# medical-genomics-group/ci-gwas

Hardware: AMD Instinct MI355X
Metric: ci_tests_per_sec (higher is better)
Workload: dtype f32; 1 GPU; cusk level sweep, one LD block 10000 SNPs x 20 traits, N=16384, alpha=0.0001, max level 5 (north_star headline); correlation matrix from synthetic .bed (Kendall-npn/Pearson) resident in HBM; n_variables=10020, engine=cusk

## Files before the change

ci-gwas_amd/csrc/cusk_internal.h:

```cpp
#pragma once
#include <hip/hip_runtime.h>

#include <cstdint>
#include <cstdio>
#include <string>
#include <vector>

#include "../../include/cusk_hip.h"

namespace cusk {

constexpr int kML = CUSK_ML;
constexpr int kLevels = CUSK_ML + 2;
constexpr unsigned long long kNone = ~0ull;
constexpr int kNumClasses = 5;
constexpr int kClassCap[kNumClasses] = {39, 63, 127, 191, 1 << 30};
constexpr int kThreads = 256;
constexpr int kTmajMinLevelDefault = 6;
constexpr int kCounterSlots = 512;
constexpr size_t kLdsLimit = 160 * 1024;

struct DevBuf
{
    void *p = nullptr;
// ... 75 lines not shown

    int n = 0;
    int words = 0;
    int mode = -1;
    bool have_result = false;
    cusk::DevBuf adj, adj0;
    cusk::DevBuf deg, binom, counters, slots, rec_base, ti, queue, symflag;
    cusk::DevBuf off[2], nbr[2], best[2];
    cusk::DevBuf planblk;
    unsigned plan_seq = 0;
    cusk::DevBuf off1;
    cusk::DevBuf items[2][cusk::kNumClasses];
    cusk::DevBuf rec_x, rec_y, rec_l, rec_s;
    long long rec_cap = 0;
    long long rec_slots = 0;
    cusk::DevBuf den_x, den_y, den_l, den_z, den_s, den_counts, den_off;
    long long den_stride = 0;
    bool records_ready = false, z_ready = false;
    cusk::DevBuf scratch_a, scratch_b;
    const float *last_C = nullptr;
    int last_levels = 0;
    std::vector<int> batch_lo, batch_hi;
    cusk::DevBuf row_range, row_blk, blk_woff;
    cusk::PinnedBuf batch_pinned;
    cusk::PinnedBuf res_pinned;
    cusk::DevBuf rv, rpos, sel, wpre;
    cusk::DevBuf nv;
    int level1_form = -1;
    long long nrec = 0;
    cusk::LevelCounters *hcnt = nullptr;
    unsigned long long *hslots = nullptr;
    long long *hrec_base = nullptr;
    unsigned long long *hcanon = nullptr;
    int *hflag = nullptr;
    std::vector<unsigned long long> binom_host;
    long long binom_rows = 0;
    cusk::HostGate *hgate = nullptr, *hgate_dev = nullptr;
    int run_seq = 0;
    long long item_cap_cur = 0;
    hipEvent_t ev_main[2] = {nullptr, nullptr};
    hipEvent_t ev_run[2] = {nullptr, nullptr};
    hipEvent_t ev_k0[cusk::kLevels], ev_k1[cusk::kLevels], ev_l0[cusk::kLevels], ev_l1[cusk::kLevels];

    int opt_fast = 1;
    int opt_validate = 0;
    int opt_het_filter = 0;
    int opt_het_rows = 0;
    int opt_corr_fp4 = 1;
    int opt_pair = 1;
    int opt_rows = 1;
    int opt_vec = 1;
    int opt_overlap = 1;
    int opt_corr_popcount = 0;
    int opt_corr_mxp_f32 = 0;
    int opt_assume_symmetric = 0;
    long long opt_queue_cap = 4ll << 20;
    int opt_hostprof = 0;
    int opt_tmaj_validate_stride = 1;
    int opt_max_staged_classes = -1;
    int opt_tmaj_min_level = cusk::kTmajMinLevelDefault;
    long long opt_chunk = 2048;
    long long opt_chunk0 = 512;
    long long opt_chunk0_low = 256;
    int opt_vec_threads = 64;
    long long opt_item_cap = 1ll << 20;
    int opt_lookahead = 2;
    int opt_sync2 = 1;
    int opt_l1_threads = 0;
    int opt_l1_lds_row = 1;
    int opt_timing = 1;
    long long opt_sep_ws_budget = 4ll << 30;

    int shard_rank = 0, shard_world = 1;
    int shard_host_staging = 0;
    cusk_exchange_fn shard_fn = nullptr;
    void *shard_user = nullptr;
    cusk::PinnedBuf shard_host;

    cusk::DevBuf bed_dev, phen_dev, mean_dev, std_dev, planes, mxp_dev, pxp_dev, mxp_bq;
    cusk::DevBuf pc_masks, pc_counts;
    cusk::DevBuf mp_bits;
    cusk::DevBuf corr_tab[2];
    cusk::PinnedBuf corr_tab_pinned[2];
    hipEvent_t ev_corr[5] = {nullptr, nullptr, nullptr, nullptr, nullptr};
    float corr_ms[4] = {0, 0, 0, 0};
    float prune_ms[5] = {0, 0, 0, 0, 0};
    float ord_ms[3] = {0, 0, 0};
    hipEvent_t ev_prune[6] = {nullptr, nullptr, nullptr, nullptr, nullptr, nullptr};
    float phen_ms[5] = {0, 0, 0, 0, 0};
};

namespace cusk {

inline int fail(cusk_engine *e, int code, const std::string &msg)
{
    if (e) e->err = msg;
    return code;
}

#define CUSK_HIP(e, call)                                                                        \
// ... 48 lines not shown
```

ci-gwas_amd/csrc/engine.hip:

```cpp
#include <algorithm>
#include <cstdlib>
#include <cstring>

#include "sweep_common.h"

using namespace cusk;


extern "C" int cusk_engine_create(cusk_engine **out, int device, void *stream)
{
    if (!out) return CUSK_ERR_ARG;
    *out = nullptr;
    int ndev = 0;
    if (hipGetDeviceCount(&ndev) != hipSuccess || ndev <= 0)
    {
        std::fprintf(stderr, "libcusk_hip: no HIP device available (this library has no CPU fallback)\n");
        return CUSK_ERR_HIP;
    }
    if (device < 0 || device >= ndev) return CUSK_ERR_ARG;
    if (hipSetDevice(device) != hipSuccess) return CUSK_ERR_HIP;
    cusk_engine *e = new cusk_engine();
    e->device = device;
    for (int l = 0; l < kLevels; l++) e->ev_k0[l] = e->ev_k1[l] = e->ev_l0[l] = e->ev_l1[l] = nullptr;
    bool ok = true;
    if (stream)
    {
        e->stream = reinterpret_cast<hipStream_t>(stream);
        e->own_stream = false;
    }
    else
    {
        ok = ok && hipStreamCreateWithFlags(&e->stream, hipStreamNonBlocking) == hipSuccess;
        e->own_stream = ok;
    }
    ok = ok && hipStreamCreateWithFlags(&e->stream2, hipStreamNonBlocking) == hipSuccess;
    ok = ok && hipStreamCreateWithFlags(&e->stream3, hipStreamNonBlocking) == hipSuccess;
    ok = ok && hipEventCreateWithFlags(&e->ev_fork, hipEventDisableTiming) == hipSuccess;
    ok = ok && hipEventCreateWithFlags(&e->ev_join, hipEventDisableTiming) == hipSuccess;
    ok = ok && hipEventCreateWithFlags(&e->ev_z, hipEventDisableTiming) == hipSuccess;
    {
        char *hctl = nullptr;
        ok = ok && hipHostMalloc(reinterpret_cast<void **>(&hctl), kCtlBytes) == hipSuccess;
        if (ok)
        {
            e->hcnt = reinterpret_cast<LevelCounters *>(hctl + kCtlCnt);
            e->hslots = reinterpret_cast<unsigned long long *>(hctl + kCtlSlots);
            e->hrec_base = reinterpret_cast<long long *>(hctl + kCtlRecBase);
            e->hcanon = reinterpret_cast<unsigned long long *>(hctl + kCtlCanon);
        }
    }
    ok = ok && hipHostMalloc(reinterpret_cast<void **>(&e->hflag), sizeof(int)) == hipSuccess;
    ok = ok && hipHostMalloc(reinterpret_cast<void **>(&e->hgate), sizeof(HostGate) * kLevels, hipHostMallocMapped | hipHostMallocCoherent) == hipSuccess;
    if (ok)
    {
        std::memset(e->hgate, 0, sizeof(HostGate) * kLevels);
        ok = hipHostGetDevicePointer(reinterpret_cast<void **>(&e->hgate_dev), e->hgate, 0) == hipSuccess;
    }
    for (auto &ev : e->ev_run) ok = ok && hipEventCreate(&ev) == hipSuccess;
    for (auto &ev : e->ev_main) ok = ok && hipEventCreate(&ev) == hipSuccess;
    for (auto &ev : e->ev_corr) ok = ok && hipEventCreate(&ev) == hipSuccess;
    for (int l = 0; l < kLevels; l++)
    {
        ok = ok && hipEventCreate(&e->ev_k0[l]) == hipSuccess && hipEventCreate(&e->ev_k1[l]) == hipSuccess;
        ok = ok && hipEventCreate(&e->ev_l0[l]) == hipSuccess && hipEventCreate(&e->ev_l1[l]) == hipSuccess;
    }
    if (!ok)
    {
        cusk_engine_destroy(e);
        return CUSK_ERR_HIP;
    }
    *out = e;
    if (const char *env = std::getenv("CUSK_OPTIONS"))
    {
        std::string all(env);
        size_t pos = 0;
        while (pos < all.size())
        {
            const size_t end = std::min(all.find(',', pos), all.size());
            const std::string kv = all.substr(pos, end - pos);
            const size_t eq = kv.find('=');
            if (eq != std::string::npos)
// ... 74 lines not shown
    else if (k == "queue_capacity" && value > 0)
        e->opt_queue_cap = value;
    else if (k == "chunk" && value >= 256)
        e->opt_chunk = value;
    else if (k == "max_staged_classes")
        e->opt_max_staged_classes = (int)value;
    else if (k == "tmaj_validate_stride" && value >= 1 && (value & (value - 1)) == 0)
        e->opt_tmaj_validate_stride = (int)value;
    else if (k == "tmaj_min_level")
        e->opt_tmaj_min_level = (int)value;
    else if (k == "hostprof")
        e->opt_hostprof = (int)value;
    else if (k == "chunk0_low" && value >= 64)
        e->opt_chunk0_low = value;
    else if (k == "chunk0" && value >= 64)
        e->opt_chunk0 = value;
    else if (k == "vec_threads" && (value == 64 || value == 128 || value == 256))
        e->opt_vec_threads = (int)value;
    else if (k == "item_capacity" && value > 0)
    {
        e->opt_item_cap = value;
        e->item_cap_cur = 0;
    }
    else if (k == "lookahead" && value >= 0)
        e->opt_lookahead = (int)value;
    else if (k == "timing")
        e->opt_timing = (int)value;
    else if (k == "l1_threads" && (value == 0 || value == 256 || value == 512))
        e->opt_l1_threads = (int)value;
    else if (k == "l1_lds_row" && (value == 0 || value == 1))
        e->opt_l1_lds_row = (int)value;
    else if (k == "sync2")
        e->opt_sync2 = (int)value;
    else if (k == "sepselect_ws_bytes" && value > 0)
        e->opt_sep_ws_budget = value;
    else
        return fail(e, CUSK_ERR_ARG, "unknown option " + k);
    return CUSK_OK;
}

extern "C" int cusk_engine_set_row_shard(cusk_engine *e, int rank, int world, cusk_exchange_fn fn, void *user, int host_staging)
{
    if (!e) return CUSK_ERR_ARG;
    if (world < 1 || rank < 0 || rank >= world || (world > 1 && !fn))
        return fail(e, CUSK_ERR_ARG, "cusk_engine_set_row_shard: need 0 <= rank < world and an exchange function");
    e->shard_rank = rank;
    e->shard_world = world;
    e->shard_fn = fn;
    e->shard_user = user;
    e->shard_host_staging = host_staging ? 1 : 0;
    return CUSK_OK;
}

extern "C" const char *cusk_last_error(const cusk_engine *e) { return e ? e->err.c_str() : "no engine"; }
extern "C" void *cusk_engine_stream(const cusk_engine *e) { return e ? (void *)e->stream : nullptr; }
extern "C" int cusk_engine_device(const cusk_engine *e) { return e ? e->device : -1; }
extern "C" int cusk_engine_level1_form(const cusk_engine *e) { return e ? e->level1_form : -1; }
extern "C" int cusk_engine_bind_thread(cusk_engine *e)
{
    if (!e) return CUSK_ERR_ARG;
    CUSK_HIP(e, hipSetDevice(e->device));
    return CUSK_OK;
}

static RunArgs skeleton_args(const float *C_dev, const float *N_dev, const float *Th, int n, int maxlevel)
{
// ... 465 lines not shown
```

ci-gwas_amd/csrc/level_loop.hip:

```cpp
#include <algorithm>
#include <atomic>
#include <chrono>

#include "host/level_policy.h"
#include "sweep_common.h"

namespace cusk {
namespace {

#define STEP(call) do { const int rc_ = (call); if (rc_ != CUSK_OK) return rc_; } while (0)

struct LevelPlan
{
    SweepParams sp;
    FinalizeParams fp;
    long long nitems[kNumClasses];
    bool use_pair = false, use_fast = false, use_rows = false, filter_ok = true;
    size_t pair_lds = 0;
    bool redone = false;
    bool known_items = false;
    int maxdeg_bound = 0;
    int staged_classes = 0;
    unsigned long long chunk0 = 0;
    bool tmaj = false;
// ... 6 lines not shown
    bool het0;
    bool het0_exact;
    bool sharded;
    bool batched;
    bool ness_checked;
    bool ness_checked_rows;
};

struct LevelRun
{
    cusk_engine *e;
    const RunArgs &a;
    hipStream_t s = e->stream;
    const int n = a.n, words = (n + 63) / 64, last_level = std::min(kML, a.maxlevel);
    ModeFlags m = {};
    cusk_stats local = {};
    long long &item_cap = e->item_cap_cur;
    int run_seq = 0, staged_classes = 0, lookahead = 0;
    char *ctl = nullptr;
    LevelCounters *dcnt = nullptr;
    unsigned long long *dslots = nullptr, *dcanon = nullptr;
    int *dsym = nullptr;
    LevelPlan plan[kLevels];
    PlanArgs pa;
    unsigned long long qcap_gate[kLevels];
    unsigned long long chunk = 0, chunk0 = 0;
    bool symmetric = false, rows_timed = false, first_pass = true;
    bool ness_symmetric = false;
    int level1_form = -1;
    int maxdeg1 = 0, maxdeg2 = -1;
    int start = 1;
    int redo = 0;
    int enq_last = 0, planned_last = 0;
    bool closed = false, done = false;
    int level_out = (a.maxlevel < 0) ? 0 : last_level + 1, levels_swept = 0;
    const std::chrono::steady_clock::time_point hp_t0 = std::chrono::steady_clock::now();
    std::string hp_log;

    void hp_mark(const char *what)
    {
        if (!e->opt_hostprof) return;
        const double us = std::chrono::duration<double, std::micro>(std::chrono::steady_clock::now() - hp_t0).count();
        char buf[64];
        std::snprintf(buf, sizeof(buf), " %s=%.1f", what, us);
        hp_log += buf;
    }
    void mark_redone(int l) { plan[l].redone = true; local.exact_fallbacks++; qcap_gate[l] = ~0ull; }
    int *off_of(int l) const { return (l == 1) ? e->off1.as<int>() : e->off[l & 1].as<int>(); }
    float level_threshold(int l) const { return m.het ? a.Th[0] : (a.mode == 0) ? a.Th[l] : uniform_ess_threshold(a.Th[0], a.ess_uniform, l); }

    int prepare()
    {
        CUSK_HIP(e, hipSetDevice(e->device));
        for (auto &q : qcap_gate) q = ~0ull;
        e->n = n;
        e->words = words;
        e->mode = a.mode;
        e->have_result = false;
        e->nrec = 0;
        e->level1_form = -1;
        m.het = (a.Ness != nullptr);
        m.het0 = m.het && a.mode == 0;
        m.het0_exact = m.het0 && e->opt_het_filter == 0;
        m.sharded = e->shard_world > 1;
        m.batched = (a.row_range != nullptr);
        m.ness_checked = m.het0 && e->opt_het_filter != 0 && last_level >= 2;
// ... 72 lines not shown
        local.max_degree[0] = n - 1;
        local.edges[0] = (long long)n * (n - 1);
        local.tests[0] = m.batched ? a.level0_pairs : (long long)n * (n - 1) / 2;
        local.canonical_tests[0] = local.tests[0];
        local.levels_run = 1;
        if (last_level >= 1 && !m.batched)
            CUSK_HIP(e, launch_degree(e->adj.as<unsigned long long>(), e->deg.as<int>(), n, words,
                                      a.mode == 0 ? e->adj0.as<unsigned long long>() : nullptr, s));
        return CUSK_OK;
    }

    int launch_sweeps(int l, bool exact_only)
    {
        LevelPlan &pl = plan[l];
        SweepParams sp = pl.sp;
        if (pl.use_rows && !exact_only)
        {
            CUSK_HIP(e, launch_level1_rows(a.mode, e->opt_validate != 0, pl.filter_ok && e->opt_fast != 0, sp, e->rv.as<float>(),
                                           e->rpos.p, e->sel.as<unsigned>(), e->wpre.as<int>(), e->opt_timing ? e->ev_main[0] : nullptr,
                                           e->opt_timing ? e->ev_main[1] : nullptr, e->shard_rank, e->shard_world, e->opt_l1_threads, e->opt_l1_lds_row != 0, m.sharded,
                                           a.time_index != nullptr, (a.mode == 1) ? dcanon + (size_t)l * kCounterSlots : nullptr, s,
                                           m.het0 ? e->nv.as<float>() : nullptr, &level1_form));
            rows_timed = true;
            return CUSK_OK;
        }
        if (l == 1) level1_form = (pl.use_pair && !exact_only) ? 1 : 0;
        bool may[kNumClasses];
        const int nonempty = classes_with_work(pl.known_items, pl.nitems, pl.staged_classes, pl.maxdeg_bound, kClassCap, kNumClasses, may);
        const bool fork = (nonempty > 1) && (e->opt_overlap != 0);
        if (fork)
        {
            CUSK_HIP(e, hipEventRecord(e->ev_fork, s));
            CUSK_HIP(e, hipStreamWaitEvent(e->stream2, e->ev_fork, 0));
        }
        bool first = true;
        for (int c = 0; c < kNumClasses; c++)
        {
            if (!may[c]) continue;
            hipStream_t cs = (fork && !first) ? e->stream2 : s;
            first = false;
            sp.items = e->items[l & 1][c].as<int2>();
            sp.cap = kClassCap[c];
            sp.cls = c;
            sp.chunk = (c == 0) ? pl.chunk0 : chunk;
            sp.item_cap = item_cap;
            sp.grid_cap = item_cap;
            if (l >= 2 && !pl.use_pair && !pl.tmaj)
            {
                const int dmax = std::min(pl.maxdeg_bound, kClassCap[c]);
                const unsigned long long sets = binom_sat(dmax, l);
                const unsigned long long per_row = sets / sp.chunk + 1ull;
                if (per_row < (1ull << 40)) sp.grid_cap = std::min<long long>(item_cap, (long long)(per_row * (unsigned long long)n));
            }
            sp.validate = e->opt_validate ? std::max(1, e->opt_tmaj_validate_stride) : 0;
            switch (sweep_kind(l, c, m.het, pl.use_pair, pl.tmaj, pl.use_fast, exact_only, e->opt_vec != 0, e->opt_validate != 0,
                               c < kNumClasses - 1 && sweep_vec_lds_bytes(c) <= kLdsLimit, kNumClasses, kVecMaxLevel))
            {
            case SweepKind::Pair: CUSK_HIP(e, launch_pair(a.mode, sp, pl.pair_lds, cs)); break;
            case SweepKind::Tmaj: CUSK_HIP(e, launch_sweep_tmaj(a.mode, m.het, l, sp, c, cs)); break;
            case SweepKind::Vec: CUSK_HIP(e, launch_sweep_vec(a.mode, l, sp, c, c == 0 ? e->opt_vec_threads : kThreads, cs)); break;
            case SweepKind::Fast: CUSK_HIP(e, launch_sweep_fast(a.mode, m.het, l, e->opt_validate != 0, sp, c, cs)); break;
            case SweepKind::Exact: CUSK_HIP(e, launch_sweep_exact(a.mode, m.het, l, sp, c, cs)); break;
            }
        }
        if (fork)
        {
// ... 84 lines not shown
        pl.redone = false;
        pl.known_items = false;
        const bool first_build = (l == 1 && first_pass);
        pa.deg = e->deg.as<int>();
        pa.off = off_of(l);
        for (int c = 0; c < kNumClasses; c++) pa.items[c] = e->items[cs][c].as<int2>();
        pa.n = n;
        pa.L = l;
        pa.binom = e->binom.as<unsigned long long>();
        pa.chunk = chunk;
        const float th_l = level_threshold(l);
        const bool vec0 = (e->opt_fast != 0) && l >= 2 && l < kVecMaxLevel && th_l >= kThMinFilter && !m.het && e->opt_vec &&
                          !e->opt_validate && staged_classes > 0;
        const unsigned long long c0 = (l <= 4) ? (unsigned long long)std::max<long long>(e->opt_chunk0_low, 64) : chunk0;
        pl.chunk0 = vec0 ? c0 : chunk;
        pl.tmaj = (e->opt_fast != 0) && !pl.force_exact && l >= std::max(2, e->opt_tmaj_min_level) && l <= kML &&
                  th_l >= kThMinFilter && (!m.het || (m.ness_checked && ness_symmetric)) && symmetric && !m.sharded;
        if (pl.tmaj) pl.chunk0 = chunk;
        pa.chunk0 = pl.chunk0;
        pa.Lsets = pl.tmaj ? l + 1 : l;
        pa.staged_classes = staged_classes;
        pa.pair_mode = ((l == 1) && !first_build && pl.use_pair && !pl.use_rows) ? 1 : 0;
        pa.cnt = dcnt + l;
        pa.prev = (l >= 2) ? dcnt + (l - 1) : nullptr;
        pa.prev_qcap = (l >= 2) ? qcap_gate[l - 1] : ~0ull;
        pa.item_cap = item_cap;
        pa.shard_rank = e->shard_rank;
        pa.shard_world = e->shard_world;
        pa.gate = e->hgate_dev + l;
        pa.seq = run_seq;
        pa.sym = (l == 1 && !e->opt_assume_symmetric && !m.batched) ? dsym : nullptr;
        pa.blocks = e->planblk.as<unsigned long long>();
        pa.blk_seq = ++e->plan_seq;
        if (first_build && e->binom_rows <= 0)
        {
            CUSK_HIP(e, e->binom.ensure(sizeof(unsigned long long) * kBinomStride));
            pa.binom = e->binom.as<unsigned long long>();
        }
        CUSK_HIP(e, launch_plan(pa, s));
        planned_last = l;
        return CUSK_OK;
    }

    int size_from_level1()
    {
        LevelPlan &pl = plan[1];
        hp_mark("plan1_enq");
        int *const rec_l_before = (a.mode == 0) ? e->rec_l.as<int>() : nullptr;
        const size_t rec_l_cleared = rec_l_before ? e->rec_l.cap : 0;
        if (rec_l_cleared) CUSK_HIP(e, hipMemsetAsync(rec_l_before, 0, rec_l_cleared, s));
        STEP(wait_gate(1));
        hp_mark("gate1");
        symmetric = (e->hgate[1].sym == 0) || (e->opt_assume_symmetric != 0) || m.batched;
        ness_symmetric = (*reinterpret_cast<volatile int *>(e->hflag) == 0);
        const long long cap_edges = std::max<long long>(e->hgate[1].total_edges, 1);
        maxdeg1 = e->hgate[1].maxdeg;
        for (int k = 0; k < 2; k++)
        {
            CUSK_HIP(e, e->nbr[k].ensure(sizeof(int) * ((size_t)cap_edges + 4)));
            if (a.mode == 0) CUSK_HIP(e, e->best[k].ensure(sizeof(unsigned long long) * (size_t)cap_edges));
        }
        CUSK_HIP(e, e->rv.ensure(sizeof(float) * ((size_t)cap_edges + 4)));
        CUSK_HIP(e, e->rpos.ensure(sizeof(int) * 4 * (size_t)cap_edges));
        CUSK_HIP(e, e->sel.ensure(sizeof(unsigned) * (size_t)cap_edges));
        if (a.mode == 0)
        {
// ... 116 lines not shown
        fp.deg = sp.deg;
        fp.words = words;
        fp.binom = sp.binom;
        fp.off1 = e->off1.as<int>();
        fp.wpre1 = e->wpre.as<int>();
        fp.adj0 = e->adj0.as<unsigned long long>();
        fp.rec_x = e->rec_x.as<int>();
        fp.rec_y = e->rec_y.as<int>();
        fp.rec_l = e->rec_l.as<int>();
        fp.rec_s = e->rec_s.as<int>();
        fp.rec_cap = e->rec_cap;
        fp.meta = pl.use_rows ? e->rpos.as<int4>() : nullptr;
        fp.cnt = dcnt + l;
        fp.slots = sp.slots;
        fp.canon = dcanon + (size_t)l * kCounterSlots;
        return CUSK_OK;
    }

    int enqueue_sweeps(int l, bool exact_only)
    {
        const bool timed = !exact_only && (e->opt_timing == 1 || e->opt_timing == 2);
        if (exact_only) mark_redone(l);
        if (timed) CUSK_HIP(e, hipEventRecord(e->ev_k0[l], s));
        STEP(launch_sweeps(l, exact_only));
        if (timed) CUSK_HIP(e, hipEventRecord(e->ev_k1[l], s));
        if (m.sharded && !exact_only) STEP(shard_join(l));
        STEP(launch_finalize(l));
        if (e->opt_timing == 2) CUSK_HIP(e, hipEventRecord(e->ev_l1[l], s));
        return CUSK_OK;
    }

    int read_back()
    {
        CUSK_HIP(e, hipEventRecord(e->ev_join, e->stream2));
        CUSK_HIP(e, hipStreamWaitEvent(s, e->ev_join, 0));
        CUSK_HIP(e, hipMemcpyAsync(e->hcnt, ctl, kCtlSym, hipMemcpyDeviceToHost, s));
        CUSK_HIP(e, hipEventRecord(e->ev_run[1], s));
        hp_mark("all_enq");
        CUSK_HIP(e, hipStreamSynchronize(s));
        hp_mark("synced");
        return CUSK_OK;
    }

    int decide_after_read_back()
    {
        int ended = 0;
        for (int l = 1; l <= planned_last && !ended; l++)
            if (!e->hcnt[l].active) ended = l;
        const int last_ran = ended ? ended - 1 : enq_last;
        const ReadBack rb = after_read_back(ended, last_ran, m.sharded, plan[last_ran].use_fast && !plan[last_ran].redone, plan[last_ran].tmaj,
                                            e->hcnt[last_ran].qcount > (unsigned long long)e->opt_queue_cap, e->hcnt[ended].overflow != 0,
                                            e->hcnt[ended].item_overflow != 0);
        long long need;
        switch (rb.what)
        {
        case AfterReadBack::Done:
            levels_swept = last_ran;
            if (ended) level_out = ended - 1;
            done = true;
            return CUSK_OK;
        case AfterReadBack::BinomOverflow:
            return fail(e, CUSK_ERR_OVERFLOW,
                        "C(degree, level) exceeds 2^62 at level " + std::to_string(ended) + " (max degree " +
                            std::to_string(e->hcnt[ended].maxdeg) + ")");
        case AfterReadBack::ReplanTmaj:
            plan[rb.level].force_exact = true;
            local.exact_fallbacks++;
            start = rb.level;
            break;
// ... 114 lines not shown
```

ci-gwas_amd/csrc/plan.hip:

```cpp
#include "sweep_common.h"

namespace cusk {


__global__ void degree_kernel(const unsigned long long *__restrict__ adj, int *deg, int n, int words, unsigned long long *adj0)
{
    const int row = blockIdx.x * (blockDim.x >> 6) + (threadIdx.x >> 6);
    const int lane = threadIdx.x & 63;
    if (row >= n) return;
    int d = 0;
    for (int w = lane; w < words; w += 64)
    {
        const unsigned long long v = adj[(size_t)row * words + w];
        if (adj0) adj0[(size_t)row * words + w] = v;
        d += __popcll(v);
    }
    for (int o = 32; o > 0; o >>= 1) d += __shfl_xor(d, o);
    if (lane == 0) deg[row] = d;
}

hipError_t launch_degree(const unsigned long long *adj, int *deg, int n, int words, unsigned long long *adj0, hipStream_t st)
{
    hipLaunchKernelGGL(degree_kernel, dim3((n + 3) / 4), dim3(256), 0, st, adj, deg, n, words, adj0);
    return hipGetLastError();
}

__global__ void fill_nbr_kernel(const unsigned long long *__restrict__ adj, const int *__restrict__ off, int *nbr,
                                unsigned long long *best, int n, int words, int *wpre, const LevelCounters *cnt,
                                const int2 *__restrict__ row_range)
{
    const int row = blockIdx.x * (blockDim.x >> 6) + (threadIdx.x >> 6);
    const int lane = threadIdx.x & 63;
// ... 46 lines not shown
    for (int i0 = 0; i0 < first; i0 += 256 * 16)
    {
        int t[16];
#pragma unroll
        for (int u = 0; u < 16; u++)
        {
            const int i = i0 + u * 256 + tid;
            t[u] = (i < first) ? in[i] : 0;
        }
#pragma unroll
        for (int u = 0; u < 16; u++) before += t[u];
    }
    int incl = v;
    for (int o = 1; o < 64; o <<= 1)
    {
        const int t = __shfl_up(incl, o);
        if (lane >= o) incl += t;
    }
    for (int o = 32; o > 0; o >>= 1) before += __shfl_xor(before, o);
    if (lane == 63) s_red[wave] = incl;
    if (lane == 0) s_red[4 + wave] = before;
    __syncthreads();
    long long pre = s_red[4] + s_red[5] + s_red[6] + s_red[7];
    for (int w = 0; w < wave; w++) pre += s_red[w];
    *block_total = s_red[0] + s_red[1] + s_red[2] + s_red[3];
    (void)n;
    return pre + incl - v;
}

constexpr int kPlanWords = 8;
static_assert(kNumClasses + 1 < 7, "plan words");
constexpr unsigned long long kPlanMask = (1ull << 40) - 1ull;

__global__ void __launch_bounds__(256) plan_kernel(PlanArgs a)
{
    __shared__ long long s_wave[kNumClasses][4];
    __shared__ int s_wdeg[4], s_wmax[4];
    __shared__ long long s_part[4][kPlanWords];
    __shared__ long long s_base[kNumClasses];
    __shared__ int s_cls[256], s_nch[256], s_pos[256];
    __shared__ unsigned long long s_big[4];
    LevelCounters *cnt = a.cnt;
    const int n = a.n, L = a.L;
    if (a.prev != nullptr && !level_complete(a.prev, a.prev_qcap))
    {
        if (blockIdx.x == 0 && threadIdx.x == 0)
        {
            HostGate *g = a.gate;
            g->active = 0;
            g->maxdeg = 0;
            g->overflow = 0;
            g->item_overflow = 0;
            g->sym = 0;
            g->total_edges = 0;
            for (int c = 0; c < kNumClasses; c++) g->class_items[c] = 0;
            __threadfence_system();
            *(volatile int *)&g->seq = a.seq;
        }
        return;
    }
    const int tid = threadIdx.x;
    const int row = blockIdx.x * 256 + tid;
    const int lane = tid & 63, wave = tid >> 6;
    int cls = -1, nchunks = 0;
    const int d = (row < n) ? a.deg[row] : 0;
    bool ovf = false;
    if (d > L)
    {
        const unsigned long long nc = a.pair_mode ? (unsigned long long)d * (d - 1) / 2
                                                  : (L == 1 ? (unsigned long long)d : a.binom[(size_t)d * kBinomStride + a.Lsets]);
        if (nc >= (1ull << 62))
            ovf = true;
        else
        {
            cls = 0;
            while (d > kClassCap[cls]) cls++;
            if (cls >= a.staged_classes) cls = kNumClasses - 1;
            const unsigned long long ch = (cls == 0) ? a.chunk0 : a.chunk;
            if (a.Lsets == L + 1 && L >= 2)
            {
                const int np = L - 2;
                long long tot = 0;
                for (int s = np; s <= d - 3; s++)
                {
                    const unsigned long long nP = (np == 0) ? 1ull : a.binom[(size_t)s * kBinomStride + np];
                    const unsigned long long per = (unsigned long long)kThreads * tmaj_prefixes_per_lane(d, s, ch);
                    tot += (long long)((nP + per - 1ull) / per);
                }
                if (tot > (long long)0x7fffffff)
                    ovf = true;
                else
                    nchunks = (int)tot;
            }
            else
            {
                const unsigned long long units = (nc + ch - 1) / ch;
                if (units > 0x7fffffffull)
                    ovf = true;
                else
                    nchunks = (int)units;
            }
            if (ovf || !(a.shard_world == 1 || row % a.shard_world == a.shard_rank))
            {
                cls = -1;
                nchunks = 0;
            }
        }
    }
    const bool wave_ovf = __ballot(ovf) != 0ull;
    int dincl = d, dmax = d;
    for (int o = 1; o < 64; o <<= 1)
    {
        const int t = __shfl_up(dincl, o);
        if (lane >= o) dincl += t;
    }
    for (int o = 32; o > 0; o >>= 1) dmax = max(dmax, __shfl_xor(dmax, o));
    if (lane == 63) s_wdeg[wave] = dincl;
    if (lane == 0) s_wmax[wave] = dmax | (wave_ovf ? (1 << 30) : 0);
    long long excl[kNumClasses];
#pragma unroll
    for (int c = 0; c < kNumClasses; c++)
    {
        const long long mine = (cls == c) ? nchunks : 0;
        long long v = mine;
        for (int o = 1; o < 64; o <<= 1)
        {
            const long long t = __shfl_up(v, o);
            if (lane >= o) v += t;
        }
        excl[c] = v - mine;
        if (lane == 63) s_wave[c][wave] = v;
    }
    __syncthreads();
    unsigned long long *blk = a.blocks + (size_t)blockIdx.x * kPlanWords;
    const unsigned long long tag = (unsigned long long)a.blk_seq << 40;
    if (tid < kPlanWords)
    {
        unsigned long long v = 0;
        if (tid == 0)
            v = (unsigned long long)((long long)s_wdeg[0] + s_wdeg[1] + s_wdeg[2] + s_wdeg[3]);
        else if (tid <= kNumClasses)
            v = (unsigned long long)(s_wave[tid - 1][0] + s_wave[tid - 1][1] + s_wave[tid - 1][2] + s_wave[tid - 1][3]);
// ... 58 lines not shown
            pos = (int)(s_base[cls] + add + e);
        }
        const bool big = (pos >= 0 && nchunks > 1);
        if (pos >= 0 && nchunks == 1) a.items[cls][pos] = make_int2(row, 0);
        const unsigned long long bm = __ballot(big);
        if (lane == 0) s_big[wave] = bm;
        if (big)
        {
            s_cls[tid] = cls;
            s_nch[tid] = nchunks;
            s_pos[tid] = pos;
        }
        __syncthreads();
        const int row0 = blockIdx.x * 256;
        for (int w = 0; w < 4; w++)
        {
            unsigned long long m = s_big[w];
            while (m)
            {
                const int r = w * 64 + __builtin_ctzll(m);
                m &= m - 1;
                const int nch = s_nch[r];
                int2 *dst = a.items[s_cls[r]] + s_pos[r];
                for (int c = tid; c < nch; c += 256) dst[c] = make_int2(row0 + r, c);
            }
        }
    }
    if (last && tid == 0)
    {
        const long long edges = before[0] + s_wdeg[0] + s_wdeg[1] + s_wdeg[2] + s_wdeg[3];
        const int maxdeg = (int)max(before[6], (long long)(max(max(s_wmax[0], s_wmax[1]), max(s_wmax[2], s_wmax[3])) & ~(1 << 30)));
        a.off[n] = (int)edges;
        const int ovf_all = (before[7] != 0 || (((s_wmax[0] | s_wmax[1] | s_wmax[2] | s_wmax[3]) >> 30) & 1)) ? 1 : 0;
        cnt->overflow = ovf_all;
        bool fits = true;
        HostGate *g = a.gate;
        for (int c = 0; c < kNumClasses; c++)
        {
            fits = fits && (tot_items[c] <= a.item_cap);
            cnt->class_items[c] = tot_items[c];
            g->class_items[c] = tot_items[c];
        }
        const int active = (maxdeg - 1 >= L && ovf_all == 0 && fits) ? 1 : 0;
        cnt->maxdeg = maxdeg;
        cnt->total_edges = edges;
        cnt->item_overflow = fits ? 0 : 1;
        cnt->active = active;
        g->active = active;
        g->maxdeg = maxdeg;
        g->overflow = ovf_all;
        g->item_overflow = fits ? 0 : 1;
        g->sym = a.sym ? *a.sym : 0;
        g->total_edges = edges;
        __threadfence_system();
        *(volatile int *)&g->seq = a.seq;
    }
}

hipError_t launch_plan(const PlanArgs &a, hipStream_t st)
{
    hipLaunchKernelGGL(plan_kernel, dim3((a.n + 255) / 256), dim3(256), 0, st, a);
    return hipGetLastError();
}

}
```

ci-gwas_amd/csrc/sweep_common.h:

```cpp
#pragma once
#include "cusk_internal.h"

namespace cusk {

constexpr int kBinomStride = 16;
constexpr int kVecMaxLevel = 9;
constexpr float kThMinFilter = 2e-3f;

struct RowInfo
{
    int cls;
    int base;
    int nchunks;
    int pad;
};

struct RecheckEntry
{
    int x;
    int k2;
    unsigned long long rank;
};

struct LevelCounters
// ... 204 lines not shown
    const unsigned long long k = chunk / ((unsigned long long)kThreads * (pairs ? pairs : 1ull));
    return (int)(k < 1ull ? 1ull : (k > 64ull ? 64ull : k));
}
hipError_t launch_sweep_vec(int mode, int L, const SweepParams &p, int cls, int threads, hipStream_t st);
unsigned persistent_grid(const void *kernel, int threads, size_t lds);
size_t sweep_vec_lds_bytes(int cls);
hipError_t launch_level0(const float *C, const float *Ness, const int *Ginit, unsigned long long *adj, int n, int words,
                         float th, int *asym_flag, hipStream_t st);
hipError_t launch_level0_batch(const float *C, const float *Ness, unsigned long long *adj, unsigned long long *adj0, int *deg, int n,
                               int words, const int2 *row_range, float th, hipStream_t st);
hipError_t launch_degree(const unsigned long long *adj, int *deg, int n, int words, unsigned long long *adj0, hipStream_t st);
hipError_t launch_fill_nbr(const unsigned long long *adj, const int *off, int *nbr, unsigned long long *best, int n, int words,
                           int *wpre, const LevelCounters *cnt, const int2 *row_range, hipStream_t st);
struct PlanArgs
{
    const int *deg;
    int *off;
    int2 *items[kNumClasses];
    int n, L;
    int Lsets;
    const unsigned long long *binom;
    unsigned long long chunk, chunk0;
    int staged_classes, pair_mode;
    LevelCounters *cnt;
    const LevelCounters *prev;
    unsigned long long prev_qcap;
    long long item_cap;
    int shard_rank, shard_world;
    HostGate *gate;
    int seq;
    const int *sym;
    unsigned long long *blocks;
    unsigned blk_seq;
};
hipError_t launch_plan(const PlanArgs &a, hipStream_t st);
hipError_t launch_expand_records(const int *rec_s, const int *rec_l, long long rec_cap, long long count, int *out,
                                 hipStream_t st);
hipError_t launch_level1_rows(int mode, bool validate, bool use_filter, const SweepParams &p, float *rv, void *meta,
                              unsigned *sel, const int *wpre, hipEvent_t ev_begin, hipEvent_t ev_end, int shard_rank,
                              int shard_world, int force_threads, bool lds_row, bool defer_apply, bool has_ti,
                              unsigned long long *canon, hipStream_t st, float *nv = nullptr, int *form = nullptr);
hipError_t launch_marks_from_bitmap(const SweepParams &p, unsigned *sel, hipStream_t st);
hipError_t launch_level1_apply(const SweepParams &p, const unsigned *sel, const void *meta, bool count_removed, hipStream_t st);
hipError_t launch_pair(int mode, const SweepParams &p, size_t lds, hipStream_t st);
hipError_t launch_gather_sub(const float *M, int n, const int *idx, int k, float *out, hipStream_t st);
hipError_t launch_gather_rows(const float *M, int n, const int *idx, const int *row_src, const int *row_k, const long long *row_first,
                              const long long *row_out, long long nrows, float *out, hipStream_t st);
hipError_t launch_pack_block_bits(const unsigned long long *adj, int n, int words, const int2 *row_range, const int *row_blk,
                                  const long long *blk_woff, unsigned long long *out, int tail, hipStream_t st);
hipError_t launch_expand_adj(const unsigned long long *adj, int *G, int n, int words, hipStream_t st);
hipError_t launch_expand_pmax(const unsigned long long *adj, const unsigned long long *adj0, const float *C, float *pmax,
                              int n, int words, const int *x, const int *y, const float *z, long long nrec, hipStream_t st);

}
```

Measured before the change: 251.8 billion CI tests/s.

## Add single-block plan kernel and kernel-based control readback via mapped host memory

```diff
diff --git a/ci-gwas_amd/csrc/cusk_internal.h b/ci-gwas_amd/csrc/cusk_internal.h
--- a/ci-gwas_amd/csrc/cusk_internal.h
+++ b/ci-gwas_amd/csrc/cusk_internal.h
@@ -131,6 +131,7 @@
     unsigned long long *hslots = nullptr;
     long long *hrec_base = nullptr;
     unsigned long long *hcanon = nullptr;
+    void *hctl_dev = nullptr;
     int *hflag = nullptr;
     std::vector<unsigned long long> binom_host;
     long long binom_rows = 0;
@@ -165,6 +166,7 @@
     long long opt_item_cap = 1ll << 20;
     int opt_lookahead = 2;
     int opt_sync2 = 1;
+    int opt_plan_one = 0;
     int opt_l1_threads = 0;
     int opt_l1_lds_row = 1;
     int opt_timing = 1;
diff --git a/ci-gwas_amd/csrc/engine.hip b/ci-gwas_amd/csrc/engine.hip
--- a/ci-gwas_amd/csrc/engine.hip
+++ b/ci-gwas_amd/csrc/engine.hip
@@ -40,13 +40,14 @@
     ok = ok && hipEventCreateWithFlags(&e->ev_z, hipEventDisableTiming) == hipSuccess;
     {
         char *hctl = nullptr;
-        ok = ok && hipHostMalloc(reinterpret_cast<void **>(&hctl), kCtlBytes) == hipSuccess;
+        ok = ok && hipHostMalloc(reinterpret_cast<void **>(&hctl), kCtlBytes, hipHostMallocMapped | hipHostMallocCoherent) == hipSuccess;
         if (ok)
         {
             e->hcnt = reinterpret_cast<LevelCounters *>(hctl + kCtlCnt);
             e->hslots = reinterpret_cast<unsigned long long *>(hctl + kCtlSlots);
             e->hrec_base = reinterpret_cast<long long *>(hctl + kCtlRecBase);
             e->hcanon = reinterpret_cast<unsigned long long *>(hctl + kCtlCanon);
+            ok = hipHostGetDevicePointer(&e->hctl_dev, hctl, 0) == hipSuccess;
         }
     }
     ok = ok && hipHostMalloc(reinterpret_cast<void **>(&e->hflag), sizeof(int)) == hipSuccess;
@@ -187,6 +188,8 @@
         e->opt_l1_lds_row = (int)value;
     else if (k == "sync2")
         e->opt_sync2 = (int)value;
+    else if (k == "plan_one" && (value == 0 || value == 1))
+        e->opt_plan_one = (int)value;
     else if (k == "sepselect_ws_bytes" && value > 0)
         e->opt_sep_ws_budget = value;
     else
diff --git a/ci-gwas_amd/csrc/level_loop.hip b/ci-gwas_amd/csrc/level_loop.hip
--- a/ci-gwas_amd/csrc/level_loop.hip
+++ b/ci-gwas_amd/csrc/level_loop.hip
@@ -62,6 +62,7 @@
     int start = 1;
     int redo = 0;
     int enq_last = 0, planned_last = 0;
+    bool forked = false;
     bool closed = false, done = false;
     int level_out = (a.maxlevel < 0) ? 0 : last_level + 1, levels_swept = 0;
     const std::chrono::steady_clock::time_point hp_t0 = std::chrono::steady_clock::now();
@@ -200,6 +201,7 @@
         {
             CUSK_HIP(e, hipEventRecord(e->ev_fork, s));
             CUSK_HIP(e, hipStreamWaitEvent(e->stream2, e->ev_fork, 0));
+            forked = true;
         }
         bool first = true;
         for (int c = 0; c < kNumClasses; c++)
@@ -350,6 +352,7 @@
         pa.sym = (l == 1 && !e->opt_assume_symmetric && !m.batched) ? dsym : nullptr;
         pa.blocks = e->planblk.as<unsigned long long>();
         pa.blk_seq = ++e->plan_seq;
+        pa.plan_one = e->opt_plan_one;
         if (first_build && e->binom_rows <= 0)
         {
             CUSK_HIP(e, e->binom.ensure(sizeof(unsigned long long) * kBinomStride));
@@ -532,9 +535,13 @@
 
     int read_back()
     {
-        CUSK_HIP(e, hipEventRecord(e->ev_join, e->stream2));
-        CUSK_HIP(e, hipStreamWaitEvent(s, e->ev_join, 0));
-        CUSK_HIP(e, hipMemcpyAsync(e->hcnt, ctl, kCtlSym, hipMemcpyDeviceToHost, s));
+        if (forked)
+        {
+            CUSK_HIP(e, hipEventRecord(e->ev_join, e->stream2));
+            CUSK_HIP(e, hipStreamWaitEvent(s, e->ev_join, 0));
+            forked = false;
+        }
+        CUSK_HIP(e, launch_ctl_mirror(ctl, e->hctl_dev, kCtlSym, s));
         CUSK_HIP(e, hipEventRecord(e->ev_run[1], s));
         hp_mark("all_enq");
         CUSK_HIP(e, hipStreamSynchronize(s));
diff --git a/ci-gwas_amd/csrc/plan.hip b/ci-gwas_amd/csrc/plan.hip
--- a/ci-gwas_amd/csrc/plan.hip
+++ b/ci-gwas_amd/csrc/plan.hip
@@ -1,3 +1,5 @@
+#include <algorithm>
+
 #include "sweep_common.h"
 
 namespace cusk {
@@ -110,6 +112,105 @@
 static_assert(kNumClasses + 1 < 7, "plan words");
 constexpr unsigned long long kPlanMask = (1ull << 40) - 1ull;
 
+struct PlanRow
+{
+    int cls, nchunks;
+    bool ovf;
+};
+
+__device__ __forceinline__ unsigned long long plan_binom(const PlanArgs &a, int d)
+{
+    const bool need = (d > a.L) && !a.pair_mode && a.L != 1;
+    return a.binom[(size_t)(need ? d : 0) * kBinomStride + a.Lsets];
+}
+
+__device__ __forceinline__ PlanRow plan_row(const PlanArgs &a, int row, int d, unsigned long long cdl)
+{
+    const int L = a.L;
+    PlanRow r = {-1, 0, false};
+    if (d <= L) return r;
+    const unsigned long long nc = a.pair_mode ? (unsigned long long)d * (d - 1) / 2 : (L == 1 ? (unsigned long long)d : cdl);
+    if (nc >= (1ull << 62))
+    {
+        r.ovf = true;
+        return r;
+    }
+    int cls = 0;
+    while (d > kClassCap[cls]) cls++;
+    if (cls >= a.staged_classes) cls = kNumClasses - 1;
+    const unsigned long long ch = (cls == 0) ? a.chunk0 : a.chunk;
+    int nchunks = 0;
+    if (a.Lsets == L + 1 && L >= 2)
+    {
+        const int np = L - 2;
+        long long tot = 0;
+        for (int s = np; s <= d - 3; s++)
+        {
+            const unsigned long long nP = (np == 0) ? 1ull : a.binom[(size_t)s * kBinomStride + np];
+            const unsigned long long per = (unsigned long long)kThreads * tmaj_prefixes_per_lane(d, s, ch);
+            tot += (long long)((nP + per - 1ull) / per);
+        }
+        if (tot > (long long)0x7fffffff)
+            r.ovf = true;
+        else
+            nchunks = (int)tot;
+    }
+    else
+    {
+        const unsigned long long units = (nc + ch - 1) / ch;
+        if (units > 0x7fffffffull)
+            r.ovf = true;
+        else
+            nchunks = (int)units;
+    }
+    if (r.ovf || !(a.shard_world == 1 || row % a.shard_world == a.shard_rank)) return r;
+    r.cls = cls;
+    r.nchunks = nchunks;
+    return r;
+}
+
+__device__ __forceinline__ void plan_close_gate(const PlanArgs &a)
+{
+    HostGate *g = a.gate;
+    g->active = 0;
+    g->maxdeg = 0;
+    g->overflow = 0;
+    g->item_overflow = 0;
+    g->sym = 0;
+    g->total_edges = 0;
+    for (int c = 0; c < kNumClasses; c++) g->class_items[c] = 0;
+    __threadfence_system();
+    *(volatile int *)&g->seq = a.seq;
+}
+
+__device__ __forceinline__ void plan_publish(const PlanArgs &a, long long edges, int maxdeg, int ovf_all, const long long *tot_items)
+{
+    LevelCounters *cnt = a.cnt;
+    a.off[a.n] = (int)edges;
+    cnt->overflow = ovf_all;
+    bool fits = true;
+    HostGate *g = a.gate;
+    for (int c = 0; c < kNumClasses; c++)
+    {
+        fits = fits && (tot_items[c] <= a.item_cap);
+        cnt->class_items[c] = tot_items[c];
+        g->class_items[c] = tot_items[c];
+    }
+    const int active = (maxdeg - 1 >= a.L && ovf_all == 0 && fits) ? 1 : 0;
+    cnt->maxdeg = maxdeg;
+    cnt->total_edges = edges;
+    cnt->item_overflow = fits ? 0 : 1;
+    cnt->active = active;
+    g->active = active;
+    g->maxdeg = maxdeg;
+    g->overflow = ovf_all;
+    g->item_overflow = fits ? 0 : 1;
+    g->sym = a.sym ? *a.sym : 0;
+    g->total_edges = edges;
+    __threadfence_system();
+    *(volatile int *)&g->seq = a.seq;
+}
+
 __global__ void __launch_bounds__(256) plan_kernel(PlanArgs a)
 {
     __shared__ long long s_wave[kNumClasses][4];
@@ -118,74 +219,19 @@
     __shared__ long long s_base[kNumClasses];
     __shared__ int s_cls[256], s_nch[256], s_pos[256];
     __shared__ unsigned long long s_big[4];
-    LevelCounters *cnt = a.cnt;
-    const int n = a.n, L = a.L;
+    const int n = a.n;
     if (a.prev != nullptr && !level_complete(a.prev, a.prev_qcap))
     {
-        if (blockIdx.x == 0 && threadIdx.x == 0)
-        {
-            HostGate *g = a.gate;
-            g->active = 0;
-            g->maxdeg = 0;
-            g->overflow = 0;
-            g->item_overflow = 0;
-            g->sym = 0;
-            g->total_edges = 0;
-            for (int c = 0; c < kNumClasses; c++) g->class_items[c] = 0;
-            __threadfence_system();
-            *(volatile int *)&g->seq = a.seq;
-        }
+        if (blockIdx.x == 0 && threadIdx.x == 0) plan_close_gate(a);
         return;
     }
     const int tid = threadIdx.x;
     const int row = blockIdx.x * 256 + tid;
     const int lane = tid & 63, wave = tid >> 6;
-    int cls = -1, nchunks = 0;
     const int d = (row < n) ? a.deg[row] : 0;
-    bool ovf = false;
-    if (d > L)
-    {
-        const unsigned long long nc = a.pair_mode ? (unsigned long long)d * (d - 1) / 2
-                                                  : (L == 1 ? (unsigned long long)d : a.binom[(size_t)d * kBinomStride + a.Lsets]);
-        if (nc >= (1ull << 62))
-            ovf = true;
-        else
-        {
-            cls = 0;
-            while (d > kClassCap[cls]) cls++;
-            if (cls >= a.staged_classes) cls = kNumClasses - 1;
-            const unsigned long long ch = (cls == 0) ? a.chunk0 : a.chunk;
-            if (a.Lsets == L + 1 && L >= 2)
-            {
-                const int np = L - 2;
-                long long tot = 0;
-                for (int s = np; s <= d - 3; s++)
-                {
-                    const unsigned long long nP = (np == 0) ? 1ull : a.binom[(size_t)s * kBinomStride + np];
-                    const unsigned long long per = (unsigned long long)kThreads * tmaj_prefixes_per_lane(d, s, ch);
-                    tot += (long long)((nP + per - 1ull) / per);
-                }
-                if (tot > (long long)0x7fffffff)
-                    ovf = true;
-                else
-                    nchunks = (int)tot;
-            }
-            else
-            {
-                const unsigned long long units = (nc + ch - 1) / ch;
-                if (units > 0x7fffffffull)
-                    ovf = true;
-                else
-                    nchunks = (int)units;
-            }
-            if (ovf || !(a.shard_world == 1 || row % a.shard_world == a.shard_rank))
-            {
-                cls = -1;
-                nchunks = 0;
-            }
-        }
-    }
-    const bool wave_ovf = __ballot(ovf) != 0ull;
+    const PlanRow pr = plan_row(a, row, d, plan_binom(a, d));
+    const int cls = pr.cls, nchunks = pr.nchunks;
+    const bool wave_ovf = __ballot(pr.ovf) != 0ull;
     int dincl = d, dmax = d;
     for (int o = 1; o < 64; o <<= 1)
     {
@@ -310,35 +356,219 @@
         const int maxdeg = (int)max(before[6], (long long)(max(max(s_wmax[0], s_wmax[1]), max(s_wmax[2], s_wmax[3])) & ~(1 << 30)));
         a.off[n] = (int)edges;
         const int ovf_all = (before[7] != 0 || (((s_wmax[0] | s_wmax[1] | s_wmax[2] | s_wmax[3]) >> 30) & 1)) ? 1 : 0;
-        cnt->overflow = ovf_all;
-        bool fits = true;
-        HostGate *g = a.gate;
+        plan_publish(a, edges, maxdeg, ovf_all, tot_items);
+    }
+}
+
+constexpr int kPlanOneThreads = 1024, kPlanOneWaves = kPlanOneThreads / 64;
+constexpr int kPlanOneRows = 16;
+constexpr int kPlanOneMaxRows = kPlanOneThreads * kPlanOneRows;
+constexpr int kPlanSelfItems = 8;
+constexpr int kPlanSums = 1 + kNumClasses;
+constexpr size_t kPlanOneStatic = 1024;
+
+__global__ void __launch_bounds__(kPlanOneThreads) plan_one_kernel(PlanArgs a, int list_cap)
+{
+    extern __shared__ int2 s_row[];
+    __shared__ long long s_sum[kPlanSums][kPlanOneWaves];
+    __shared__ int s_max[kPlanOneWaves];
+    __shared__ int s_nlist;
+    static_assert(sizeof(s_sum) + sizeof(s_max) + sizeof(int) <= kPlanOneStatic, "static LDS of plan_one_kernel");
+    const int n = a.n;
+    int4 *const s_list = reinterpret_cast<int4 *>(s_row + ((n + 1) & ~1));
+    const int tid = threadIdx.x, lane = tid & 63, wave = tid >> 6;
+    if (a.prev != nullptr && !level_complete(a.prev, a.prev_qcap))
+    {
+        if (tid == 0) plan_close_gate(a);
+        return;
+    }
+    const int R = (n + kPlanOneThreads - 1) / kPlanOneThreads;
+    const int row0 = tid * R, row1 = min(n, row0 + R);
+    bool ovf = false;
+    {
+        int d[kPlanOneRows];
+        unsigned long long cdl[kPlanOneRows];
+#pragma unroll
+        for (int u = 0; u < kPlanOneRows; u++)
+        {
+            const int i = u * kPlanOneThreads + tid;
+            d[u] = (i < n) ? a.deg[i] : 0;
+        }
+#pragma unroll
+        for (int u = 0; u < kPlanOneRows; u++) cdl[u] = (u < R) ? plan_binom(a, d[u]) : 0ull;
+#pragma unroll
+        for (int u = 0; u < kPlanOneRows; u++)
+        {
+            const int i = u * kPlanOneThreads + tid;
+            if (i < n)
+            {
+                const PlanRow pr = plan_row(a, i, d[u], cdl[u]);
+                ovf = ovf || pr.ovf;
+                s_row[i] = make_int2(d[u] | ((pr.cls + 1) << 16), pr.nchunks);
+            }
+        }
+    }
+    const bool wave_ovf = __ballot(ovf) != 0ull;
+    __syncthreads();
+    long long mine[kPlanSums];
+#pragma unroll
+    for (int k = 0; k < kPlanSums; k++) mine[k] = 0;
+    int dmax = 0;
+    for (int row = row0; row < row1; row++)
+    {
+        const int2 v = s_row[row];
+        const int d = v.x & 0xffff, cls = (v.x >> 16) - 1;
+        dmax = max(dmax, d);
+        mine[0] += d;
+#pragma unroll
+        for (int c = 0; c < kNumClasses; c++) mine[1 + c] += (cls == c) ? v.y : 0;
+    }
+    long long exclw[kPlanSums];
+#pragma unroll
+    for (int k = 0; k < kPlanSums; k++)
+    {
+        long long v = mine[k];
+        for (int o = 1; o < 64; o <<= 1)
+        {
+            const long long t = __shfl_up(v, o);
+            if (lane >= o) v += t;
+        }
+        exclw[k] = v - mine[k];
+        if (lane == 63) s_sum[k][wave] = v;
+    }
+    for (int o = 32; o > 0; o >>= 1) dmax = max(dmax, __shfl_xor(dmax, o));
+    if (lane == 0) s_max[wave] = dmax | (wave_ovf ? (1 << 30) : 0);
+    if (tid == 0) s_nlist = 0;
+    __syncthreads();
+    long long o0 = 0;
+    long long pos[kNumClasses];
+    long long tot[kPlanSums];
+#pragma unroll
+    for (int k = 0; k < kPlanSums; k++)
+    {
+        const long long x = (lane < kPlanOneWaves) ? s_sum[k][lane] : 0;
+        long long xi = x;
+        for (int o = 1; o < kPlanOneWaves; o <<= 1)
+        {
+            const long long y = __shfl_up(xi, o);
+            if (lane >= o) xi += y;
+        }
+        const long long pre = __shfl(xi - x, wave), t = __shfl(xi, kPlanOneWaves - 1);
+        tot[k] = t;
+        if (k == 0)
+            o0 = pre + exclw[0];
+        else
+            pos[k - 1] = (t > a.item_cap) ? -1 : pre + exclw[k];
+    }
+    if (tid == 0)
+    {
+        int m = 0, maxdeg = 0;
+        for (int w = 0; w < kPlanOneWaves; w++)
+        {
+            m |= s_max[w];
+            maxdeg = max(maxdeg, s_max[w] & ~(1 << 30));
+        }
+        long long tot_items[kNumClasses];
+        for (int c = 0; c < kNumClasses; c++) tot_items[c] = tot[1 + c];
+        plan_publish(a, tot[0], maxdeg, (m >> 30) & 1, tot_items);
+    }
+    for (int r = 0; r < R; r++)
+    {
+        const int row = row0 + r;
+        int2 v = make_int2(0, 0);
+        if (row < row1)
+        {
+            v = s_row[row];
+            a.off[row] = (int)o0;
+        }
+        const int d = v.x & 0xffff, cls = (v.x >> 16) - 1, nch = v.y;
+        o0 += d;
+        long long p = -1;
+#pragma unroll
         for (int c = 0; c < kNumClasses; c++)
-        {
-            fits = fits && (tot_items[c] <= a.item_cap);
-            cnt->class_items[c] = tot_items[c];
-            g->class_items[c] = tot_items[c];
-        }
-        const int active = (maxdeg - 1 >= L && ovf_all == 0 && fits) ? 1 : 0;
-        cnt->maxdeg = maxdeg;
-        cnt->total_edges = edges;
-        cnt->item_overflow = fits ? 0 : 1;
-        cnt->active = active;
-        g->active = active;
-        g->maxdeg = maxdeg;
-        g->overflow = ovf_all;
-        g->item_overflow = fits ? 0 : 1;
-        g->sym = a.sym ? *a.sym : 0;
-        g->total_edges = edges;
-        __threadfence_system();
-        *(volatile int *)&g->seq = a.seq;
+            if (cls == c && pos[c] >= 0)
+            {
+                p = pos[c];
+                pos[c] += nch;
+            }
+        bool big = (p >= 0 && nch > kPlanSelfItems);
+        const unsigned long long bm = __ballot(big);
+        if (bm)
+        {
+            int base = 0;
+            if (lane == 0) base = atomicAdd(&s_nlist, __popcll(bm));
+            base = __shfl(base, 0);
+            const int at = base + __popcll(bm & ((1ull << lane) - 1ull));
+            if (big && at < list_cap)
+                s_list[at] = make_int4(row, cls, (int)p, nch);
+            else
+                big = false;
+        }
+        if (p >= 0 && !big)
+        {
+            int2 *dst = a.items[cls] + p;
+            for (int c = 0; c < nch; c++) dst[c] = make_int2(row, c);
+        }
+    }
+    __syncthreads();
+    const int nlist = min(s_nlist, list_cap);
+    for (int e = wave; e < nlist; e += kPlanOneWaves)
+    {
+        const int4 it = s_list[e];
+        int2 *dst = a.items[it.y] + it.z;
+        for (int c = lane; c < it.w; c += 64) dst[c] = make_int2(it.x, c);
     }
 }
 
 hipError_t launch_plan(const PlanArgs &a, hipStream_t st)
 {
-    hipLaunchKernelGGL(plan_kernel, dim3((a.n + 255) / 256), dim3(256), 0, st, a);
+    if (a.plan_one && a.n <= kPlanOneMaxRows)
+    {
+        const size_t rows = sizeof(int2) * (size_t)((a.n + 1) & ~1);
+        const size_t list_cap = std::min<size_t>((size_t)a.n, (kLdsLimit - kPlanOneStatic - rows) / sizeof(int4));
+        const size_t lds = rows + list_cap * sizeof(int4);
+        if (lds > 64 * 1024)
+        {
+            const hipError_t e = hipFuncSetAttribute(reinterpret_cast<const void *>(plan_one_kernel), hipFuncAttributeMaxDynamicSharedMemorySize, (int)lds);
+            if (e != hipSuccess) return e;
+        }
+        hipLaunchKernelGGL(plan_one_kernel, dim3(1), dim3(kPlanOneThreads), lds, st, a, (int)list_cap);
+    }
+    else
+        hipLaunchKernelGGL(plan_kernel, dim3((a.n + 255) / 256), dim3(256), 0, st, a);
     return hipGetLastError();
 }
 
-}
+
+constexpr int kMirrorThreads = 1024, kMirrorPerThread = 4;
+
+__global__ void __launch_bounds__(kMirrorThreads) ctl_mirror_kernel(const uint4 *__restrict__ src, uint4 *__restrict__ dst, unsigned n16)
+{
+    const unsigned i0 = blockIdx.x * (kMirrorThreads * kMirrorPerThread) + threadIdx.x;
+    uint4 v[kMirrorPerThread];
+#pragma unroll
+    for (int u = 0; u < kMirrorPerThread; u++)
+    {
+        const unsigned i = i0 + u * kMirrorThreads;
+        if (i < n16) v[u] = src[i];
+    }
+#pragma unroll
+    for (int u = 0; u < kMirrorPerThread; u++)
+    {
+        const unsigned i = i0 + u * kMirrorThreads;
+        if (i < n16) dst[i] = v[u];
+    }
+    __threadfence_system();
+}
+
+hipError_t launch_ctl_mirror(const void *ctl, void *dst, size_t bytes, hipStream_t st)
+{
+    const unsigned n16 = (unsigned)(bytes / 16);
+    if (n16 == 0) return hipSuccess;
+    const unsigned per = kMirrorThreads * kMirrorPerThread;
+    hipLaunchKernelGGL(ctl_mirror_kernel, dim3((n16 + per - 1) / per), dim3(kMirrorThreads), 0, st, reinterpret_cast<const uint4 *>(ctl),
+                       reinterpret_cast<uint4 *>(dst), n16);
+    return hipGetLastError();
+}
+
+}
diff --git a/ci-gwas_amd/csrc/sweep_common.h b/ci-gwas_amd/csrc/sweep_common.h
--- a/ci-gwas_amd/csrc/sweep_common.h
+++ b/ci-gwas_amd/csrc/sweep_common.h
@@ -260,8 +260,10 @@
     const int *sym;
     unsigned long long *blocks;
     unsigned blk_seq;
+    int plan_one;
 };
 hipError_t launch_plan(const PlanArgs &a, hipStream_t st);
+hipError_t launch_ctl_mirror(const void *ctl, void *dst, size_t bytes, hipStream_t st);
 hipError_t launch_expand_records(const int *rec_s, const int *rec_l, long long rec_cap, long long count, int *out,
                                  hipStream_t st);
 hipError_t launch_level1_rows(int mode, bool validate, bool use_filter, const SweepParams &p, float *rv, void *meta,
```

Measured after the change: 255.0 billion CI tests/s, median of 6. 1.3% higher.
